# lambdaloop/ucoslam-cv3

Hardware: AMD Instinct MI355X
Metric: tracking frames/sec (ORB extract + match + local BA), 1241x376 mono (higher is better)
Workload: dtype u8 (ORB, Hamming) + f64 (BA); 1 GPU; orb1241x376_2000f_8lv + hamming_knn_2000x10000_nn10 + local_ba_10kf_3000pt; frames_per_keyframe=4

## Files before the change

### ucoslam-cv3_amd/csrc/ba.hip

```cpp
#include <cfloat>
#include <functional>
#include <cstdio>
#include <emmintrin.h>
#include <immintrin.h>
#include <condition_variable>
#include <mutex>
#include <string>
#include <thread>
#include <type_traits>
#include <cmath>
#include <cstdlib>
#include <chrono>
#include <atomic>

#include "common.hpp"
#include "reduce.hpp"

namespace {

constexpr int kMaxFree = 64;
constexpr int kThreads = 256;
constexpr int kSolveThreads = 256;
constexpr int kHbmThreads = 512;
constexpr int kFusedThreads = 512;
// ... 2616 lines not shown
    ResLayout R;
    uh::Layout A;
    R.poses = A.take<float>(16 * (size_t)Kc); R.state = A.take<double>(7 * (size_t)Kc); R.points = A.take<float>(3 * (size_t)Pc);
    R.bad = A.take<unsigned char>(Ec);
    R.bytes_no_chi2 = (A.off + 7) & ~(size_t)7;
    R.chi2 = A.take<double>(Ec);
    R.bytes = (A.off + 7) & ~(size_t)7;
    return R;
}

static int ensure_staging(uh_ba* b, int K, int P, int E) {
    UH_HIP_CHECK(hipSetDevice(b->ctx->device));
    if (b->stage_in_flight) { UH_HIP_CHECK(hipEventSynchronize(b->ev_stage)); b->stage_in_flight = false; }
    if (b->h_stage && K <= b->cap_K && P <= b->cap_P && E <= b->cap_E) return UH_OK;
    const int Kc = K <= b->cap_K ? b->cap_K : K + K / 4 + 4, Pc = P <= b->cap_P ? b->cap_P : P + P / 4 + 64, Ec = E <= b->cap_E ? b->cap_E : E + E / 4 + 1024;
    const StageLayout L = stage_layout(Kc, Pc);
    const ResLayout R = res_layout(Kc, Pc, Ec);
    const size_t bytes = L.obs + (size_t)Ec * sizeof(uh_ba_obs) + 256;
    unsigned char* ns = nullptr; unsigned char* nr = nullptr;
    hipError_t e = hipHostMalloc(reinterpret_cast<void**>(&ns), bytes, hipHostMallocMapped);
    if (e == hipSuccess) e = hipHostMalloc(reinterpret_cast<void**>(&nr), R.bytes + 256, hipHostMallocMapped);
    if (e != hipSuccess) {
        if (ns) (void)hipHostFree(ns);
        uh::set_error("uh_ba: hipHostMalloc of the staging / result blocks (%zu + %zu bytes) failed: %s", bytes, R.bytes, hipGetErrorString(e));
        return UH_ENOMEM;
    }
    if (b->h_stage || b->h_res) UH_HIP_CHECK(hipStreamSynchronize(b->ctx->stream));
    if (b->h_stage) (void)hipHostFree(b->h_stage);
    if (b->h_res) (void)hipHostFree(b->h_res);
    std::memset(nr, 0, R.bytes + 256);
    b->h_stage = ns; b->h_stage_bytes = bytes; b->h_res = nr; b->h_res_bytes = R.bytes + 256;
    b->cap_K = Kc; b->cap_P = Pc; b->cap_E = Ec; b->slay = L; b->rlay = R;
    b->have_problem = false; b->optimized = false;
    if (!b->ev_stage) UH_HIP_CHECK(hipEventCreateWithFlags(&b->ev_stage, hipEventDisableTiming));
    return UH_OK;
}

struct PersistPlan { bool ok; int NF, Lw, G, krows, nelem, SL, max_fix, kfix, lds, nb4, nblk, KS, off_cam; };

template <int NF>
static int persist_lds_bytes(const PersistPlan& pl, int n) { return persist_lds<NF>(pl.krows, n, pl.max_fix, pl.kfix, pl.off_cam, pl.KS, pl.SL).total_bytes; }

static int persist_lanes(int nfree) {
    if (const char* e = getenv("UH_BA_NF")) { const int v = atoi(e); if ((v == 8 || v == 16) && nfree <= v) return v; }
    return nfree <= 8 ? 8 : (nfree <= 16 ? 16 : 0);
}

template <int NF>
static hipError_t persist_grant_lds(int bytes) {
    return hipFuncSetAttribute(reinterpret_cast<const void*>(&ba_persist_kernel<NF>), hipFuncAttributeMaxDynamicSharedMemorySize, bytes);
}

static PersistPlan plan_persistent(uh_ba* b, int K, int P, int E, int nfree) {
    PersistPlan pl{};
    const char* form = getenv("UH_BA_FORM");
    if (form && std::string(form) == "legacy") return pl;
    if (getenv("UH_BA_WIDE") && atoi(getenv("UH_BA_WIDE")) != 0) return pl;
    void* dflag = nullptr;
    if (!b->h_stop || hipHostGetDevicePointer(&dflag, b->h_stop, 0) != hipSuccess) return pl;
    if (nfree < 1 || P < 1 || E >= (1 << 20) - 1) return pl;
    if (b->persist_blocked > 0) { --b->persist_blocked; return pl; }
    const int NF = persist_lanes(nfree);
    if (!NF) return pl;
    const int kLwMax = kPThreads / NF;
    int Lw = std::max(std::min(8, kLwMax), std::min(kLwMax, uh_div_up(P, 64)));
    if (const char* e = getenv("UH_BA_LW")) Lw = std::max(1, std::min(kLwMax, atoi(e)));
    const int G = uh_div_up(P, Lw);
    const int cus = b->ctx->num_cus > 0 ? b->ctx->num_cus : 256;
    if (G > cus) return pl;
    const int kfix = K - nfree;
    if (kfix > 255) return pl;
    pl.NF = NF; pl.Lw = Lw; pl.G = G; pl.kfix = kfix;
    pl.max_fix = Lw * kfix;
    pl.krows = (3 * Lw + 15) & ~15;
    const int n = 6 * nfree;
    pl.nb4 = (n + 3) / 4; pl.nblk = pl.nb4 * (pl.nb4 + 1) / 2;
    pl.off_cam = pl.nblk * 16;
    pl.nelem = pl.off_cam + NF * 27 + 6 * NF + 4;
    pl.SL = (uh_div_up(pl.nelem, G) + 1) & ~1;
    pl.KS = 1;
    {
        int best = 1 << 30;
        for (int ks = 1; ks <= 6; ks++) {
            if (ks > 1 && ks * pl.off_cam > (n + 1) * (n + 1) + 1452) break;
            const int rounds = uh_div_up(pl.nblk * ks, kPThreads), depth = (uh_div_up(pl.krows, ks) + 3) & ~3;
            if (rounds * depth < best) { best = rounds * depth; pl.KS = ks; }
        }
    }
    pl.lds = NF == 8 ? persist_lds_bytes<8>(pl, n) : persist_lds_bytes<16>(pl, n);
    if (b->max_lds <= 0) {
        int v = 0;
        if (hipDeviceGetAttribute(&v, hipDeviceAttributeMaxSharedMemoryPerBlock, b->ctx->device) != hipSuccess || v <= 0) v = 64 * 1024;
        b->max_lds = v;
    }
    if (pl.lds > b->max_lds) return pl;
    const int cls = NF == 8 ? 0 : 1;
    if (pl.lds > b->p_lds_set[cls]) {
        if ((NF == 8 ? persist_grant_lds<8>(pl.lds) : persist_grant_lds<16>(pl.lds)) != hipSuccess) { (void)hipGetLastError(); return pl; }
        b->p_lds_set[cls] = pl.lds;
    }
    pl.ok = true;
    return pl;
}

__attribute__((target("avx512f,avx512vl,avx512dq"))) static int pack_obs16_avx512(const int32_t* pt_, const int32_t* kf_, const float* uv_, const double* w_, int e0, int e1, int P, int K,
                                                                                 unsigned char* ob, bool& exact_out, unsigned& oob) {
    const __m256i pmax = _mm256_set1_epi32(P - 1), kmax = _mm256_set1_epi32(K - 1);
    __m256i bad = _mm256_setzero_si256();
    __mmask8 exact = 0xFF;
    const __m512i idx0 = _mm512_setr_epi32(0, 16, 17, 8, 1, 18, 19, 9, 2, 20, 21, 10, 3, 22, 23, 11);
    const __m512i idx1 = _mm512_setr_epi32(4, 24, 25, 12, 5, 26, 27, 13, 6, 28, 29, 14, 7, 30, 31, 15);
    int i = e0;
    unsigned char* dst = ob + 16 * (size_t)e0;
    for (; i + 8 <= e1; i += 8, dst += 128) {
        const __m256i pt = _mm256_loadu_si256(reinterpret_cast<const __m256i*>(pt_ + i));
        const __m256i kf = _mm256_loadu_si256(reinterpret_cast<const __m256i*>(kf_ + i));
        const __m512 uv = _mm512_loadu_ps(uv_ + 2 * i);
        const __m512d w = _mm512_loadu_pd(w_ + i);
        bad = _mm256_or_si256(bad, _mm256_or_si256(_mm256_or_si256(pt, _mm256_sub_epi32(pmax, pt)), _mm256_or_si256(kf, _mm256_sub_epi32(kmax, kf))));
        const __m256 wf = _mm512_cvtpd_ps(w);
        exact &= _mm512_cmp_pd_mask(_mm512_cvtps_pd(wf), w, _CMP_EQ_OQ);
        const __m256i pk = _mm256_or_si256(pt, _mm256_slli_epi32(kf, 24));
        const __m512 a = _mm512_insertf32x8(_mm512_castps256_ps512(_mm256_castsi256_ps(pk)), wf, 1);
        _mm512_storeu_ps(dst, _mm512_permutex2var_ps(a, idx0, uv));
        _mm512_storeu_ps(dst + 64, _mm512_permutex2var_ps(a, idx1, uv));
    }
    if (exact != 0xFF) exact_out = false;
    oob |= _mm256_movemask_ps(_mm256_castsi256_ps(bad)) ? 1u : 0u;
    return i - e0;
}

using ObsPacker = std::function<void(int, int, bool, bool&, unsigned&)>;
static int set_problem_fast(uh_ba* b, int K, int P, int E, const PersistPlan& pl, bool obs16 = false, const ObsPacker* pack = nullptr, unsigned* oob_out = nullptr) {
    const StageLayout& L = b->slay;
    unsigned char* hs = b->h_stage;
    const float* poses = reinterpret_cast<const float*>(hs + L.poses_in);
    const unsigned char* fixed = hs + L.fixed;
    const float* intr_f = reinterpret_cast<const float*>(hs + L.intr_f);
    double* pose0 = reinterpret_cast<double*>(hs + L.pose0); double* R0 = reinterpret_cast<double*>(hs + L.poseR0);
    double* intr = reinterpret_cast<double*>(hs + L.intr);
    int* slot = reinterpret_cast<int*>(hs + L.slot); int* free_kf = reinterpret_cast<int*>(hs + L.free_kf); int* fix_kf = reinterpret_cast<int*>(hs + L.fix_kf);
    int nfree = 0, nfix = 0;
    for (int k = 0; k < K; k++) {
        if (!fixed[k]) { slot[k] = nfree; free_kf[nfree++] = k; } else { slot[k] = -1; fix_kf[nfix++] = k; }
        const float* M = poses + 16 * k;
        const double R[9] = {M[0], M[1], M[2], M[4], M[5], M[6], M[8], M[9], M[10]};
        double* qq = pose0 + 7 * k;
        quat_from_R_host(R, qq);
        qq[4] = M[3]; qq[5] = M[7]; qq[6] = M[11];
        for (int j = 0; j < 4; j++) intr[4 * k + j] = intr_f[4 * k + j];
        double* Rk = R0 + 12 * k;
        const double tx = 2 * qq[0], ty = 2 * qq[1], tz = 2 * qq[2];
        const double twx = tx * qq[3], twy = ty * qq[3], twz = tz * qq[3];
        const double txx = tx * qq[0], txy = ty * qq[0], txz = tz * qq[0];
        const double tyy = ty * qq[1], tyz = tz * qq[1], tzz = tz * qq[2];
        Rk[0] = 1 - (tyy + tzz); Rk[1] = txy - twz; Rk[2] = txz + twy;
        Rk[3] = txy + twz; Rk[4] = 1 - (txx + tzz); Rk[5] = tyz - twx;
        Rk[6] = txz - twy; Rk[7] = tyz + twx; Rk[8] = 1 - (txx + tyy);
        Rk[9] = qq[4]; Rk[10] = qq[5]; Rk[11] = qq[6];
    }
    UH_HIP_CHECK(hipSetDevice(b->ctx->device));
    hipStream_t st = b->ctx->stream;
    int rc;
    if ((rc = b->dstage.reserve(b->h_stage_bytes))) return rc;
    if ((rc = b->dT.reserve((size_t)P * K * sizeof(unsigned) + 256))) return rc;
    if (b->dT_gen != b->dT.gen || (b->tseq & 0xFFFu) == 0xFFFu) {
        UH_HIP_CHECK(hipMemsetAsync(b->dT.p, 0, b->dT.cap, st));
        b->dT_gen = b->dT.gen; b->tseq = 0;
    }
// ... 568 lines not shown
```

### ucoslam-cv3_amd/csrc/ba_persist.hpp

```cpp
#pragma once

#pragma clang fp contract(fast)

constexpr int kPThreads = 256;
constexpr int kPWaves = kPThreads / 64;
constexpr long long kPTimeoutTicksDefault = 10000000ll;

struct BAPersist {
    int G, Lw, krows, SL, nelem, max_fix, kfix;
    int nb4, nblk, KS;
    int n1, n2, stop_at_begin;
    int speculate;
    unsigned launch_id;
    long long timeout_ticks;
    unsigned tag_base;
    float minChi2;
    const unsigned* T; unsigned tseq;
    const uh_ba_obs* obs;
    int obs16;
    const float* points;
    const float* poses_in;
    const int* fix_kf;
    const double* pose0; const double* poseR0;
    float* r_poses; double* r_state; float* r_points; unsigned char* r_bad; double* r_chi2;
    int want_chi2;
    unsigned long long* r_dev; unsigned long long* r_host; size_t r_words;
    unsigned* done_ctr; unsigned done_base;
    unsigned long long* part;
    unsigned long long* red;
    unsigned long long* partC;
    BAState* host_state;
    unsigned long long* host_done;
    unsigned long long* errw;
};

constexpr int kFxCam = 20;
struct PersistLds {
    int Yt, U, usz, out, wsum, x, bp, bs, bsp, wv, pose, poseR, red, sc, fxchi, fxobs, fxcam, fxact_bytes, fxk_bytes, fxid_bytes, fxptr_bytes, pair_bytes, blk_bytes, flag_bytes, total_bytes;
};
template <int NF>
__host__ __device__ inline PersistLds persist_lds(int krows, int n, int max_fix, int kfix, int off_cam, int KS, int SL) {
    constexpr int NP = 6 * NF, YS = NP + 2;
    PersistLds o;
    int a = 0;
    o.Yt = a; a += krows * YS;
    o.U = a;
    o.usz = (n + 1) * (n + 1) + (n + 1 <= 64 ? 2 * 121 * 6 : 2 * 6 * 128 + 4);
    if (o.usz < KS * off_cam) o.usz = KS * off_cam;
    { const int r = KS * off_cam + (SL > 256 ? SL : 256) + 8; if (o.usz < r) o.usz = r; }
    if (o.usz < kPWaves * NF * 33) o.usz = kPWaves * NF * 33;
    if (o.usz < 2048) o.usz = 2048;
    a += o.usz;
    o.out = a; a += NF * 27 + NP + 4;
    o.wsum = a; a += kPWaves * NF * 33;
    o.x = a; a += NP; o.bp = a; a += NP; o.bs = a; a += NP;
    o.bsp = a; a += kPWaves * NP;
    o.wv = a; a += krows;
    o.pose = a; a += 2 * NF * 7; o.poseR = a; a += 2 * NF * 12;
    o.red = a; a += 16; o.sc = a; a += 8;
    o.fxchi = a; a += max_fix;
    o.fxobs = a; a += 3 * max_fix;
    o.fxcam = a; a += kFxCam * kfix;
    o.fxact_bytes = a * 8;
    int b = o.fxact_bytes + ((max_fix + 15) & ~15);
    o.fxk_bytes = b; b += (max_fix + 15) & ~15;
    o.fxid_bytes = b; b += 4 * ((max_fix + 3) & ~3);
    o.fxptr_bytes = b; b += 4 * (kPThreads / NF + 4);
    o.pair_bytes = b; b += NF * (NF + 1) / 2 * 4;
    b = (b + 15) & ~15;
    o.blk_bytes = b; b += ((NP / 4) * (NP / 4 + 1) / 2 * 2 + 15) & ~15;
    o.flag_bytes = b; b += 16;
    o.total_bytes = b;
    return o;
}

typedef unsigned long long pword;
struct TWord { pword lo, hi; };
__device__ __forceinline__ void tst(pword* base, size_t i, double v, unsigned tag) {
    const pword b = (pword)__double_as_longlong(v);
    typedef unsigned int u32x4 __attribute__((ext_vector_type(4)));
    const u32x4 w = {(unsigned)b, tag, (unsigned)(b >> 32), tag};
    const __amdgpu_buffer_rsrc_t rs = __builtin_amdgcn_make_buffer_rsrc(base, 0, 0x7FFFFFFF, 0x00020000);
    __builtin_amdgcn_raw_buffer_store_b128(w, rs, (int)(i * 16), 0, 16);
}
__device__ __forceinline__ TWord tld_raw(const pword* base, size_t i) {
    TWord w;
    w.lo = __hip_atomic_load(base + 2 * i, __ATOMIC_RELAXED, __HIP_MEMORY_SCOPE_AGENT);
    w.hi = __hip_atomic_load(base + 2 * i + 1, __ATOMIC_RELAXED, __HIP_MEMORY_SCOPE_AGENT);
    return w;
}
__device__ __forceinline__ bool tok(const TWord& w, unsigned tag) { return (unsigned)(w.lo >> 32) == tag && (unsigned)(w.hi >> 32) == tag; }
__device__ __forceinline__ double tval(const TWord& w) { return __longlong_as_double((long long)((w.hi << 32) | (w.lo & 0xffffffffull))); }

__device__ __forceinline__ double rsqrt_nr(double x) {
    double r = __builtin_amdgcn_rsq(x);
    r = r * fma(-0.5 * x, r * r, 1.5);
    r = r * fma(-0.5 * x, r * r, 1.5);
    return r;
}

template <int JAC>
__device__ __forceinline__ void edge_eval_p(double u, double v, double w, double fx, double fy, double cx, double cy, double delta, double dsqr,
                                            const double* Rt, const double* X, bool robust, EdgeLin& o) {
    const double x = Rt[0] * X[0] + Rt[1] * X[1] + Rt[2] * X[2] + Rt[9];
    const double y = Rt[3] * X[0] + Rt[4] * X[1] + Rt[5] * X[2] + Rt[10];
    const double z = Rt[6] * X[0] + Rt[7] * X[1] + Rt[8] * X[2] + Rt[11];
    const double iz = fast_rcp(z);
    const double xz = x * iz, yz = y * iz;
    o.ex = u - (xz * fx + cx);
    o.ey = v - (yz * fy + cy);
    o.chi2 = w * (o.ex * o.ex + o.ey * o.ey);
    o.rho1 = 1.0;
    o.robchi = o.chi2;
    if (robust && o.chi2 > dsqr) {
        const double rs = rsqrt_nr(o.chi2);
        o.rho1 = delta * rs;
        o.robchi = 2 * (o.chi2 * rs) * delta - dsqr;
    }
    if (JAC >= 1) {
        o.ww = o.rho1 * w;
        o.r0 = -w * o.ex * o.rho1;
        o.r1 = -w * o.ey * o.rho1;
        const double fxz = fx * iz, fyz = fy * iz;
#pragma unroll
        for (int c = 0; c < 3; c++) {
            o.A[c] = -fxz * (Rt[c] - xz * Rt[6 + c]);
            o.A[3 + c] = -fyz * (Rt[3 + c] - yz * Rt[6 + c]);
        }
        if (JAC >= 2) {
            o.B[0] = xz * yz * fx; o.B[1] = -(1 + xz * xz) * fx; o.B[2] = yz * fx; o.B[3] = -fxz; o.B[4] = 0; o.B[5] = xz * fxz;
            o.B[6] = (1 + yz * yz) * fy; o.B[7] = -xz * yz * fy; o.B[8] = -xz * fy; o.B[9] = 0; o.B[10] = -fyz; o.B[11] = yz * fyz;
        }
// ... 238 lines not shown
    for (int i = tid; i < kPWaves * NP; i += kPThreads) s_bsp[i] = 0.0;
    for (int i = tid; i < NF * 27 + NP + 4; i += kPThreads) s_out[i] = 0.0;
    for (int i = tid; i < 2 * NF * 7; i += kPThreads) s_pose[i] = 0.0;
    for (int i = tid; i < 2 * NF * 12; i += kPThreads) s_poseR[i] = 0.0;
    if (tid < 8) s_sc[tid] = 0.0;
    __syncthreads();
    if (tid < nl) {
        int c = 0;
        for (int j = 0; j < q.kfix; j++) c += cell(l0 + tid, q.fix_kf[j]) >= 0;
        s_fxptr[tid + 1] = c;
    }
    if (tid == 0) s_fxptr[0] = 0;
    __syncthreads();
    if (tid == 0) for (int i = 0; i < nl; i++) s_fxptr[i + 1] += s_fxptr[i];
    __syncthreads();
    if (tid < nl) {
        int at = s_fxptr[tid];
        for (int j = 0; j < q.kfix; j++) {
            const int e = cell(l0 + tid, q.fix_kf[j]);
            if (e < 0) continue;
            double fu, fv, fw;
            load_obs(e, fu, fv, fw);
            s_fxact[at] = 1; s_fxchi[at] = 0.0; s_fxk[at] = (unsigned char)j; s_fxid[at] = e;
            s_fxobs[3 * at] = fu; s_fxobs[3 * at + 1] = fv; s_fxobs[3 * at + 2] = fw;
            ++at;
        }
    }
    for (int i = tid; i < q.kfix * kFxCam; i += kPThreads) {
        const int f = i / kFxCam, j = i - f * kFxCam, k = q.fix_kf[f];
        s_fxcam[i] = j < 12 ? q.poseR0[12 * k + j] : (j < 16 ? p.intr[4 * k + (j - 12)] : (double)q.poses_in[16 * (size_t)k + 8 + (j - 16)]);
    }
    const int fxb = live ? s_fxptr[ll] : 0, fxe = live ? s_fxptr[ll + 1] : 0;
    if (tid < nfree) {
        const int k = p.free_kf[tid];
        for (int b = 0; b < 2; b++) {
            for (int j = 0; j < 7; j++) s_pose[(b * NF + tid) * 7 + j] = q.pose0[7 * k + j];
            for (int j = 0; j < 12; j++) s_poseR[(b * NF + tid) * 12 + j] = q.poseR0[12 * k + j];
        }
    }
    for (int t = tid; t < npairs; t += kPThreads) {
        int s1 = 0, rem = t;
        while (rem >= nfree - s1) { rem -= nfree - s1; ++s1; }
        s_pair[t][0] = (short)s1; s_pair[t][1] = (short)(s1 + rem);
    }
    for (int t = tid; t < q.nblk; t += kPThreads) {
        int bi = 0, rem = t;
        while (rem >= q.nb4 - bi) { rem -= q.nb4 - bi; ++bi; }
        s_blk[t][0] = (unsigned char)bi; s_blk[t][1] = (unsigned char)(bi + rem);
    }
    if (tid == 0) { s_flag[0] = 1; s_flag[1] = 0; s_flag[2] = 0; }
    __syncthreads();

    unsigned ep = 0, tagA = 0;
    auto next_tag = [&]() -> unsigned { ++ep; return q.tag_base | (ep & 0xFFFu); };
    const pword err_word = ((pword)q.launch_id << 32) | 1ull;
    auto give_up = [&](long long& t0) -> bool {
        if (t0 < 63) { ++t0; return false; }
        if (t0 == 63) t0 = wall_clock64();
        if (__hip_atomic_load(q.errw, __ATOMIC_RELAXED, __HIP_MEMORY_SCOPE_AGENT) == err_word || wall_clock64() - t0 > q.timeout_ticks) {
            s_flag[1] = 1;
            __hip_atomic_store(q.errw, err_word, __ATOMIC_RELAXED, __HIP_MEMORY_SCOPE_AGENT);
            if (q.host_done) __hip_atomic_store(q.host_done, ((unsigned long long)q.launch_id << 32) | 2ull, __ATOMIC_RELEASE, __HIP_MEMORY_SCOPE_SYSTEM);
            return true;
        }
        __builtin_amdgcn_s_sleep(1);
        return false;
    };
    auto tload8 = [&](const pword* base, size_t first, size_t stride, int cnt, unsigned tag, double (&v)[8], unsigned need = 0xFFu) {
        long long t0 = 0;
        for (;;) {
            TWord w[8];
            bool ok = true;
#pragma unroll
            for (int u = 0; u < 8; u++) if (u < cnt && ((need >> u) & 1u)) w[u] = tld_raw(base, first + u * stride);
#pragma unroll
            for (int u = 0; u < 8; u++) { if (u < cnt && ((need >> u) & 1u)) { ok = ok && tok(w[u], tag); v[u] = tval(w[u]); } else v[u] = 0.0; }
            if (ok || give_up(t0)) return;
        }
    };
    const unsigned sl_inv = (unsigned)(0x100000000ull / (unsigned)SL) + 1u;
    auto div_sl = [&](int i) -> int { return (int)__umulhi((unsigned)i, sl_inv); };
    auto part_at = [&](int i) -> size_t { const int sl = div_sl(i); return ((size_t)sl * G + g) * SL + (i - sl * SL); };

    auto prod_index = [&](int row, int col) -> int {
        const int bi = row >> 2, bj = col >> 2;
        return (bi * q.nb4 - bi * (bi - 1) / 2 + (bj - bi)) * 16 + (row & 3) * 4 + (col & 3);
    };
    auto is_diag_elem = [&](int idx) -> bool {
        if (idx >= OFF_CAM) return false;
        int row, col;
        const int bq = idx >> 4;
        row = 4 * s_blk[bq][0] + ((idx >> 2) & 3); col = 4 * s_blk[bq][1] + (idx & 3);
        return row == col && col < n;
    };
    int fold_i[2], fold_s[2];
#pragma unroll
    for (int u = 0; u < 2; u++) {
        const int t = tid + u * kPThreads;
        fold_i[u] = -1; fold_s[u] = 0;
        if (t < nfree * 21) {
            const int sc = t / 21, qq = t - 21 * sc;
            int a = 0, rem = qq;
            while (rem >= 6 - a) { rem -= 6 - a; ++a; }
            fold_i[u] = prod_index(6 * sc + a, 6 * sc + a + rem);
            fold_s[u] = sc * 27 + qq;
        }
    }
    const bool red_diag0 = tid < SL && is_diag_elem(g * SL + tid);
    const int open_beg = div_sl(OFF_CAM) * SL;
    const int red_HG = max(1, min(G, kPThreads / SL));
    const unsigned hg_inv = (unsigned)(0x100000000ull / (unsigned)red_HG) + 1u;
    bool clk_on = false;
    int n_kept = 0, n_dropped = 0;
#define UH_BA_CLKT(i) do { if (clk_on) UH_BA_CLK(i); } while (0)
    BAState st;
    memset(&st, 0, sizeof(st));
    st.phase = 2; st.lambda = -1; st.ni = 2;
    bool robust = true;
    double chi_lin_pass = 0;

    double acc[10];
    double hp[33];
    double H[18];
    bool any = false;
    auto lin_eval = [&](int buf, const double (&Xp)[3], bool first) {
#pragma unroll
        for (int i = 0; i < 10; i++) acc[i] = 0;
#pragma unroll
        for (int i = 0; i < 33; i++) hp[i] = 0;
#pragma unroll
        for (int i = 0; i < 18; i++) H[i] = 0;
        any = false;
        const bool on = has && act;
        if (on) {
            EdgeLin L;
            edge_eval_p<2>(ou, ov, ow, fxk, fyk, cxk, cyk, d.delta, d.dsqr, s_poseR + (buf * NF + s) * 12, Xp, robust, L);
            any = true;
            if (first) chi_e = L.chi2;
            acc[9] = L.robchi;
            acc[0] = L.ww * (L.A[0] * L.A[0] + L.A[3] * L.A[3]); acc[1] = L.ww * (L.A[0] * L.A[1] + L.A[3] * L.A[4]);
            acc[2] = L.ww * (L.A[0] * L.A[2] + L.A[3] * L.A[5]); acc[3] = L.ww * (L.A[1] * L.A[1] + L.A[4] * L.A[4]);
            acc[4] = L.ww * (L.A[1] * L.A[2] + L.A[4] * L.A[5]); acc[5] = L.ww * (L.A[2] * L.A[2] + L.A[5] * L.A[5]);
            acc[6] = L.A[0] * L.r0 + L.A[3] * L.r1; acc[7] = L.A[1] * L.r0 + L.A[4] * L.r1; acc[8] = L.A[2] * L.r0 + L.A[5] * L.r1;
#pragma unroll
            for (int a = 0; a < 6; a++)
#pragma unroll
                for (int c = 0; c < 3; c++) H[a * 3 + c] = L.ww * (L.B[a] * L.A[c] + L.B[6 + a] * L.A[3 + c]);
            int qq = 0;
#pragma unroll
            for (int a = 0; a < 6; a++)
#pragma unroll
                for (int c = a; c < 6; c++) hp[qq++] = L.ww * (L.B[a] * L.B[c] + L.B[6 + a] * L.B[6 + c]);
#pragma unroll
            for (int a = 0; a < 6; a++) hp[21 + a] = L.B[a] * L.r0 + L.B[6 + a] * L.r1;
        }
        {
            for (int i = fxb + s; i < fxe; i += NF) {
                if (!s_fxact[i]) continue;
                any = true;
                const double* C = s_fxcam + kFxCam * s_fxk[i];
                EdgeLin L;
                edge_eval_p<1>(s_fxobs[3 * i], s_fxobs[3 * i + 1], s_fxobs[3 * i + 2], C[12], C[13], C[14], C[15], d.delta, d.dsqr, C, Xp, robust, L);
                if (first) s_fxchi[i] = L.chi2;
                acc[9] += L.robchi;
                acc[0] += L.ww * (L.A[0] * L.A[0] + L.A[3] * L.A[3]); acc[1] += L.ww * (L.A[0] * L.A[1] + L.A[3] * L.A[4]);
                acc[2] += L.ww * (L.A[0] * L.A[2] + L.A[3] * L.A[5]); acc[3] += L.ww * (L.A[1] * L.A[1] + L.A[4] * L.A[4]);
                acc[4] += L.ww * (L.A[1] * L.A[2] + L.A[4] * L.A[5]); acc[5] += L.ww * (L.A[2] * L.A[2] + L.A[5] * L.A[5]);
                acc[6] += L.A[0] * L.r0 + L.A[3] * L.r1; acc[7] += L.A[1] * L.r0 + L.A[4] * L.r1; acc[8] += L.A[2] * L.r0 + L.A[5] * L.r1;
            }
        }
    };
    auto phase1 = [&](double lambda, bool first, double scale_lane, double stop_val) {
        tagA = next_tag();
        if (!first) UH_BA_CLKT(52);
#pragma unroll
        for (int i = 0; i < 10; i++) acc[i] = group_sum<NF>(acc[i]);
        const unsigned long long anym = __ballot(any);
        any_pt = ((anym >> (lane & ~(NF - 1))) & ((1ull << NF) - 1)) != 0;
        bl0 = acc[6]; bl1 = acc[7]; bl2 = acc[8];
        if (first) {
        } else if (any_pt) {
            const double d00 = acc[0] + lambda, d11 = acc[3] + lambda, d22 = acc[5] + lambda;
            ci00 = rsqrt_nr(d00);
            cl10 = acc[1] * ci00; cl20 = acc[2] * ci00;
            ci11 = rsqrt_nr(d11 - cl10 * cl10);
            cl21 = (acc[4] - cl20 * cl10) * ci11;
            ci22 = rsqrt_nr(d22 - cl20 * cl20 - cl21 * cl21);
            wl0 = bl0 * ci00;
            wl1 = (bl1 - cl10 * wl0) * ci11;
            wl2 = (bl2 - cl20 * wl0 - cl21 * wl1) * ci22;
        } else {
            ci00 = ci11 = ci22 = cl10 = cl20 = cl21 = wl0 = wl1 = wl2 = 0;
        }
        if (!first && 3 * ll + 2 < q.krows) {
#pragma unroll
            for (int a = 0; a < 6; a++) {
                const double y0 = H[a * 3] * ci00;
                const double y1 = (H[a * 3 + 1] - cl10 * y0) * ci11;
                const double y2 = (H[a * 3 + 2] - cl20 * y0 - cl21 * y1) * ci22;
                Yt[(3 * ll) * YS + 6 * s + a] = y0; Yt[(3 * ll + 1) * YS + 6 * s + a] = y1; Yt[(3 * ll + 2) * YS + 6 * s + a] = y2;
                hp[27 + a] = y0 * wl0 + y1 * wl1 + y2 * wl2;
            }
        }
        {
            int off = 0, real = 33;
            PartTranspose<33, 32, NF>::run(hp, lane, off, real);
#pragma unroll
            for (int i = 0; i < NHP; i++) if (i < real) s_wsum[(wv * NF + s) * 33 + off + i] = hp[i];
        }
        if (!first) UH_BA_CLKT(53);
        const double chi_part = (live && s == 0) ? acc[9] : 0.0;
        const double maxd = (live && s == 0 && any_pt) ? fmax(fabs(acc[0]), fmax(fabs(acc[3]), fabs(acc[5]))) : 0.0;
        double cs = chi_part, mx = maxd, ss = scale_lane;
        block_reduce3<kPWaves>(cs, mx, ss, s_red);
        for (int t = tid; t < NF * 33; t += kPThreads) {
            double r = s_wsum[t];
#pragma unroll
            for (int w = 1; w < kPWaves; w++) r += s_wsum[w * NF * 33 + t];
            const int sc = t / 33, i = t - 33 * sc;
            s_out[i < 27 ? sc * 27 + i : NF * 27 + 6 * sc + (i - 27)] = r;
        }
        if (tid == 0) { s_out[NF * 27 + NP] = cs; s_out[NF * 27 + NP + 1] = ss; s_out[NF * 27 + NP + 2] = mx; s_out[NF * 27 + NP + 3] = g == 0 ? stop_val : 0.0; }
        if (!first) UH_BA_CLKT(54);
        if (!first) {
            const int nitems = q.nblk * q.KS;
            const int kc = (q.krows + q.KS - 1) / q.KS;
            for (int item = tid; item < nitems; item += kPThreads) {
                const int kt = item / q.nblk, bq = item - kt * q.nblk;
                const int bi = s_blk[bq][0], bj = s_blk[bq][1];
                const int kbeg = kt * kc, kend = min(q.krows, kbeg + kc);
                double acc4[16];
#pragma unroll
                for (int i = 0; i < 16; i++) acc4[i] = 0;
                const double* ra = Yt + 4 * bi, * rb = Yt + 4 * bj;
                for (int k = kbeg; k < kend; k += 4) {
                    double2 a01[4], a23[4], b01[4], b23[4];
#pragma unroll
                    for (int u = 0; u < 4; u++) {
                        const int kk = k + u < kend ? k + u : kbeg;
                        a01[u] = *reinterpret_cast<const double2*>(ra + kk * YS); a23[u] = *reinterpret_cast<const double2*>(ra + kk * YS + 2);
                        b01[u] = *reinterpret_cast<const double2*>(rb + kk * YS); b23[u] = *reinterpret_cast<const double2*>(rb + kk * YS + 2);
                    }
#pragma unroll
                    for (int u = 0; u < 4; u++) {
                        const double z = k + u < kend ? 1.0 : 0.0;
                        const double av[4] = {a01[u].x * z, a01[u].y * z, a23[u].x * z, a23[u].y * z}, bv[4] = {b01[u].x, b01[u].y, b23[u].x, b23[u].y};
#pragma unroll
                        for (int r = 0; r < 4; r++)
#pragma unroll
                            for (int c = 0; c < 4; c++) acc4[r * 4 + c] = fma(av[r], bv[c], acc4[r * 4 + c]);
                    }
                }
#pragma unroll
                for (int i = 0; i < 16; i++) U[kt * OFF_CAM + bq * 16 + i] = acc4[i];
            }
        }
        if (!first) UH_BA_CLKT(55);
        __syncthreads();
        if (!first) UH_BA_CLKT(56);
        if (!first) {
#pragma unroll
            for (int u = 0; u < 2; u++) if (fold_i[u] >= 0) U[fold_i[u]] -= s_out[fold_s[u]];
            for (int j = tid; j < n; j += kPThreads) { const int sc = j / 6; s_out[NF * 27 + j] -= s_out[sc * 27 + 21 + (j - 6 * sc)]; }
        }
        __syncthreads();
        if (!first) UH_BA_CLKT(60);
        for (int i = tid; i < NF * 27 + NP + 4; i += kPThreads) {
            if (!first && i < NF * 27 && i - 27 * (i / 27) < 21) continue;
            tst(q.part, part_at(OFF_CAM + i), s_out[i], tagA);
        }
        if (!first) UH_BA_CLKT(61);
        const int KSs = q.KS;
        for (int i = (first ? open_beg : 0) + tid; i < OFF_CAM; i += kPThreads) {
            double r = 0.0;
            if (!first) { r = U[i]; for (int kt = 1; kt < KSs; kt++) r += U[kt * OFF_CAM + i]; }
            tst(q.part, part_at(i), r, tagA);
        }
    };

    unsigned tagB = 0;
    auto reduce_slices = [&](double lam, bool first) -> bool {
        tagB = next_tag();
        const int HG = red_HG;
        double* const R = U + q.KS * OFF_CAM;
        const size_t src = (size_t)g * G * SL;
        for (int idx = tid; idx < SL * HG; idx += kPThreads) {
            const int hg = div_sl(idx), e = idx - hg * SL;
            const bool is_max = g * SL + e == OFF_SC + 2;
            const int ge = g * SL + e;
            const bool hpp = ge >= OFF_CAM && ge < OFF_BS && (ge - OFF_CAM) - 27 * ((ge - OFF_CAM) / 27) < 21;
            const bool used = ge < q.nelem && !(first && (g + 1) * SL <= OFF_CAM) && !(hpp && !first);
            double r = 0.0;
            bool have = false;
            for (int h = hg; used && h < G; h += 8 * HG) {
                double v[8];
                const int cnt = min(8, HG == 1 ? G - h : (int)__umulhi((unsigned)(G - h + HG - 1), hg_inv));
                tload8(q.part, src + (size_t)h * SL + e, (size_t)HG * SL, cnt, tagA, v);
#pragma unroll
                for (int u = 0; u < 8; u++) {
                    if (u >= cnt) continue;
                    r = !have ? v[u] : (is_max ? fmax(r, v[u]) : r + v[u]);
                    have = true;
                }
            }
            R[idx] = r;
        }
        UH_BA_CLKT(50);
        __syncthreads();
        if (s_flag[1]) return false;
        for (int e = tid; e < SL; e += kPThreads) {
            const bool is_max = g * SL + e == OFF_SC + 2;
            double r = R[e];
            for (int hg = 1; hg < HG; hg++) { const double v = R[hg * SL + e]; r = is_max ? fmax(r, v) : r + v; }
            if (e == tid ? red_diag0 : is_diag_elem(g * SL + e)) r -= lam;
            {
                const int ge = g * SL + e;
                if (!first && ge >= OFF_CAM && ge < OFF_BS && (ge - OFF_CAM) - 27 * ((ge - OFF_CAM) / 27) < 21) continue;
            }
            tst(q.red, (size_t)g * SL + e, r, tagB);
        }
        UH_BA_CLKT(51);
        __syncthreads();
        return true;
    };

    auto dst_of = [&](int idx) -> int {
        int t = -1;
        if (idx < q.nelem) {
            if (idx < OFF_CAM) {
                int row, col;
                const int bq = idx >> 4, rr = (idx >> 2) & 3, cq = idx & 3;
                row = 4 * s_blk[bq][0] + rr; col = 4 * s_blk[bq][1] + cq;
                if (row <= col && col < n) t = o.U + col * ld + row;
            } else if (idx < OFF_BS) {
                const int i = idx - OFF_CAM, sc = i / 27, k = i - 27 * sc;
                if (k >= 21) t = (o.bp + 6 * sc + (k - 21)) | (1 << 24);
            } else if (idx < OFF_SC) t = o.U + n * ld + (idx - OFF_BS);
            else t = (o.sc + 4 + (idx - OFF_SC)) | (1 << 24);
        }
        return t;
    };
    int asm_dst[8];
#pragma unroll
    for (int u = 0; u < 8; u++) asm_dst[u] = dst_of(tid + u * kPThreads);
    UH_BA_CLK(1);
    for (int pass = 0; pass < 2; pass++) {
        UH_BA_CLK(2 + 3 * pass);
        if (pass == 1) {
            if (st.stopped) break;
            st.gate = 1;
            st.iters_pass1 = st.iters_done;
            if (has) {
                const double* Rt = s_poseR + (st.cur * NF + s) * 12;
                const double z = Rt[6] * X[0] + Rt[7] * X[1] + Rt[8] * X[2] + Rt[11];
                if (chi_e > d.chi2_th || !(z > 0.0)) act = false;
            }
            for (int i = fxb + s; i < fxe; i += NF) {
                const double* Rt = s_fxcam + kFxCam * s_fxk[i];
                const double z = Rt[6] * X[0] + Rt[7] * X[1] + Rt[8] * X[2] + Rt[11];
                if (s_fxchi[i] > d.chi2_th || !(z > 0.0)) s_fxact[i] = 0;
            }
            robust = false;
            __syncthreads();
        }
        const int max_iters = pass == 0 ? q.n1 : q.n2;
        st.pending = 0; st.stop_seen = 0;
        st.phase = max_iters > 0 ? 0 : 2;
// ... 302 lines not shown
```

Baseline: 9187 frames/s.

## Restructure persistent BA Schur block products into per-wave K-split with shuffle reduction

Replaces the flat item loop that wrote each K-slice of every 4x4 block product into LDS and then summed slices after a block barrier. Each wave now owns a group of blocks, with lanes split across K slices. Partial sums are combined by wavefront shuffles, staged in a small per-wave LDS buffer, and streamed straight to the global partial buffer. The camera-diagonal fold is precomputed into a compact Hb buffer during the wsum reduction, and the KS selection cost model is changed to match. The aim is to cut LDS footprint and block-wide syncs and to overlap global stores with compute; the price is more complex indexing and wave-level fences, which carry correctness risk.

```diff
diff --git a/ucoslam-cv3_amd/csrc/ba.hip b/ucoslam-cv3_amd/csrc/ba.hip
--- a/ucoslam-cv3_amd/csrc/ba.hip
+++ b/ucoslam-cv3_amd/csrc/ba.hip
@@ -2722,9 +2722,10 @@
     {
         int best = 1 << 30;
         for (int ks = 1; ks <= 6; ks++) {
-            if (ks > 1 && ks * pl.off_cam > (n + 1) * (n + 1) + 1452) break;
-            const int rounds = uh_div_up(pl.nblk * ks, kPThreads), depth = (uh_div_up(pl.krows, ks) + 3) & ~3;
-            if (rounds * depth < best) { best = rounds * depth; pl.KS = ks; }
+            const int bpw = std::min(64 / ks, uh_div_up(pl.nblk, kPWaves));
+            const int rounds = uh_div_up(pl.nblk, kPWaves * bpw), depth = (uh_div_up(pl.krows, ks) + 3) & ~3;
+            const int cost = rounds * (depth + (ks - 1) + 4);
+            if (cost < best) { best = cost; pl.KS = ks; }
         }
     }
     pl.lds = NF == 8 ? persist_lds_bytes<8>(pl, n) : persist_lds_bytes<16>(pl, n);
diff --git a/ucoslam-cv3_amd/csrc/ba_persist.hpp b/ucoslam-cv3_amd/csrc/ba_persist.hpp
--- a/ucoslam-cv3_amd/csrc/ba_persist.hpp
+++ b/ucoslam-cv3_amd/csrc/ba_persist.hpp
@@ -4,6 +4,7 @@
 
 constexpr int kPThreads = 256;
 constexpr int kPWaves = kPThreads / 64;
+constexpr bool kCameraSideFirst = false;
 constexpr long long kPTimeoutTicksDefault = 10000000ll;
 
 struct BAPersist {
@@ -36,7 +37,7 @@
 
 constexpr int kFxCam = 20;
 struct PersistLds {
-    int Yt, U, usz, out, wsum, x, bp, bs, bsp, wv, pose, poseR, red, sc, fxchi, fxobs, fxcam, fxact_bytes, fxk_bytes, fxid_bytes, fxptr_bytes, pair_bytes, blk_bytes, flag_bytes, total_bytes;
+    int Yt, U, usz, bpw, hb, rscr, out, wsum, x, bp, bs, bsp, wv, pose, poseR, red, sc, fxchi, fxobs, fxcam, fxact_bytes, fxk_bytes, fxid_bytes, fxptr_bytes, pair_bytes, blk_bytes, flag_bytes, total_bytes;
 };
 template <int NF>
 __host__ __device__ inline PersistLds persist_lds(int krows, int n, int max_fix, int kfix, int off_cam, int KS, int SL) {
@@ -46,8 +47,16 @@
     o.Yt = a; a += krows * YS;
     o.U = a;
     o.usz = (n + 1) * (n + 1) + (n + 1 <= 64 ? 2 * 121 * 6 : 2 * 6 * 128 + 4);
-    if (o.usz < KS * off_cam) o.usz = KS * off_cam;
-    { const int r = KS * off_cam + (SL > 256 ? SL : 256) + 8; if (o.usz < r) o.usz = r; }
+    {
+        const int nblk = off_cam / 16, nb4 = (n + 3) / 4, per = (nblk + kPWaves - 1) / kPWaves;
+        o.bpw = 64 / KS < per ? 64 / KS : per;
+        const int scr = (SL > 256 ? SL : 256) + 8, hbsz = 2 * nb4 * 16;
+        const int cap = o.usz > KS * off_cam + scr ? o.usz : KS * off_cam + scr;
+        while (o.bpw > 1 && kPWaves * o.bpw * 16 + hbsz + scr > cap) --o.bpw;
+        o.hb = kPWaves * o.bpw * 16;
+        o.rscr = o.hb + hbsz;
+        if (o.usz < o.rscr + scr) o.usz = o.rscr + scr;
+    }
     if (o.usz < kPWaves * NF * 33) o.usz = kPWaves * NF * 33;
     if (o.usz < 2048) o.usz = 2048;
     a += o.usz;
@@ -452,10 +461,6 @@
     auto div_sl = [&](int i) -> int { return (int)__umulhi((unsigned)i, sl_inv); };
     auto part_at = [&](int i) -> size_t { const int sl = div_sl(i); return ((size_t)sl * G + g) * SL + (i - sl * SL); };
 
-    auto prod_index = [&](int row, int col) -> int {
-        const int bi = row >> 2, bj = col >> 2;
-        return (bi * q.nb4 - bi * (bi - 1) / 2 + (bj - bi)) * 16 + (row & 3) * 4 + (col & 3);
-    };
     auto is_diag_elem = [&](int idx) -> bool {
         if (idx >= OFF_CAM) return false;
         int row, col;
@@ -463,19 +468,33 @@
         row = 4 * s_blk[bq][0] + ((idx >> 2) & 3); col = 4 * s_blk[bq][1] + (idx & 3);
         return row == col && col < n;
     };
-    int fold_i[2], fold_s[2];
-#pragma unroll
-    for (int u = 0; u < 2; u++) {
-        const int t = tid + u * kPThreads;
-        fold_i[u] = -1; fold_s[u] = 0;
-        if (t < nfree * 21) {
-            const int sc = t / 21, qq = t - 21 * sc;
+    double* const Hb = U + o.hb;
+    constexpr int NSUM = (NF * 33 + kPThreads - 1) / kPThreads, NHZ = (2 * (NP / 4) * 16 + kPThreads - 1) / kPThreads;
+    int hb_i[NSUM];
+    unsigned hb_zero = 0;
+#pragma unroll
+    for (int u = 0; u < NSUM; u++) {
+        const int t = tid + u * kPThreads, sc = t / 33, qq = t - 33 * sc;
+        hb_i[u] = -1;
+        if (sc < nfree && qq < 21) {
             int a = 0, rem = qq;
             while (rem >= 6 - a) { rem -= 6 - a; ++a; }
-            fold_i[u] = prod_index(6 * sc + a, 6 * sc + a + rem);
-            fold_s[u] = sc * 27 + qq;
-        }
-    }
+            const int row = 6 * sc + a, col = row + rem, bi = row >> 2, bj = col >> 2;
+            hb_i[u] = ((bj - bi) * q.nb4 + bi) * 16 + (row & 3) * 4 + (col & 3);
+        }
+    }
+#pragma unroll
+    for (int u = 0; u < NHZ; u++) {
+        const int t = tid + u * kPThreads;
+        if (t < 2 * q.nb4 * 16) {
+            const int dd = t >= q.nb4 * 16 ? 1 : 0, bi = (t >> 4) - dd * q.nb4;
+            const int row = 4 * bi + ((t >> 2) & 3), col = 4 * (bi + dd) + (t & 3);
+            if (!(row <= col && col < n && row / 6 == col / 6)) hb_zero |= 1u << u;
+        }
+    }
+    const int p_kt = lane / o.bpw, p_bl = lane - p_kt * o.bpw;
+    const int p_kc = ((q.krows + q.KS - 1) / q.KS + 3) & ~3;
+    const int p_kbeg = min(q.krows, p_kt * p_kc), p_kend = p_kt < q.KS ? min(q.krows, p_kbeg + p_kc) : p_kbeg;
     const bool red_diag0 = tid < SL && is_diag_elem(g * SL + tid);
     const int open_beg = div_sl(OFF_CAM) * SL;
     const int red_HG = max(1, min(G, kPThreads / SL));
@@ -583,76 +602,127 @@
         const double maxd = (live && s == 0 && any_pt) ? fmax(fabs(acc[0]), fmax(fabs(acc[3]), fabs(acc[5]))) : 0.0;
         double cs = chi_part, mx = maxd, ss = scale_lane;
         block_reduce3<kPWaves>(cs, mx, ss, s_red);
-        for (int t = tid; t < NF * 33; t += kPThreads) {
+#pragma unroll
+        for (int u = 0; u < NSUM; u++) {
+            const int t = tid + u * kPThreads;
+            if (t >= NF * 33) break;
             double r = s_wsum[t];
 #pragma unroll
             for (int w = 1; w < kPWaves; w++) r += s_wsum[w * NF * 33 + t];
             const int sc = t / 33, i = t - 33 * sc;
-            s_out[i < 27 ? sc * 27 + i : NF * 27 + 6 * sc + (i - 27)] = r;
+            if (i < 27) {
+                s_out[sc * 27 + i] = r;
+                if (!first && hb_i[u] >= 0) Hb[hb_i[u]] = r;
+            } else {
+                if (!first && sc < nfree) {
+                    double rp = s_wsum[t - 6];
+#pragma unroll
+                    for (int w = 1; w < kPWaves; w++) rp += s_wsum[w * NF * 33 + t - 6];
+                    r -= rp;
+                }
+                s_out[NF * 27 + 6 * sc + (i - 27)] = r;
+            }
+        }
+        if (!first) {
+#pragma unroll
+            for (int u = 0; u < NHZ; u++) if ((hb_zero >> u) & 1u) Hb[tid + u * kPThreads] = 0.0;
         }
         if (tid == 0) { s_out[NF * 27 + NP] = cs; s_out[NF * 27 + NP + 1] = ss; s_out[NF * 27 + NP + 2] = mx; s_out[NF * 27 + NP + 3] = g == 0 ? stop_val : 0.0; }
+        __syncthreads();
         if (!first) UH_BA_CLKT(54);
-        if (!first) {
-            const int nitems = q.nblk * q.KS;
-            const int kc = (q.krows + q.KS - 1) / q.KS;
-            for (int item = tid; item < nitems; item += kPThreads) {
-                const int kt = item / q.nblk, bq = item - kt * q.nblk;
-                const int bi = s_blk[bq][0], bj = s_blk[bq][1];
-                const int kbeg = kt * kc, kend = min(q.krows, kbeg + kc);
-                double acc4[16];
-#pragma unroll
-                for (int i = 0; i < 16; i++) acc4[i] = 0;
-                const double* ra = Yt + 4 * bi, * rb = Yt + 4 * bj;
-                for (int k = kbeg; k < kend; k += 4) {
-                    double2 a01[4], a23[4], b01[4], b23[4];
-#pragma unroll
-                    for (int u = 0; u < 4; u++) {
-                        const int kk = k + u < kend ? k + u : kbeg;
-                        a01[u] = *reinterpret_cast<const double2*>(ra + kk * YS); a23[u] = *reinterpret_cast<const double2*>(ra + kk * YS + 2);
-                        b01[u] = *reinterpret_cast<const double2*>(rb + kk * YS); b23[u] = *reinterpret_cast<const double2*>(rb + kk * YS + 2);
-                    }
-#pragma unroll
-                    for (int u = 0; u < 4; u++) {
-                        const double z = k + u < kend ? 1.0 : 0.0;
-                        const double av[4] = {a01[u].x * z, a01[u].y * z, a23[u].x * z, a23[u].y * z}, bv[4] = {b01[u].x, b01[u].y, b23[u].x, b23[u].y};
-#pragma unroll
-                        for (int r = 0; r < 4; r++)
-#pragma unroll
-                            for (int c = 0; c < 4; c++) acc4[r * 4 + c] = fma(av[r], bv[c], acc4[r * 4 + c]);
-                    }
+        auto send_camera_side = [&]() {
+            for (int i = tid; i < NF * 27 + NP + 4; i += kPThreads) {
+                if (!first && i < NF * 27 && i - 27 * (i / 27) < 21) continue;
+                tst(q.part, part_at(OFF_CAM + i), s_out[i], tagA);
+            }
+        };
+        if (first || kCameraSideFirst) send_camera_side();
+        if (!first) UH_BA_CLKT(60);
+        if (first) {
+            for (int i = open_beg + tid; i < OFF_CAM; i += kPThreads) tst(q.part, part_at(i), 0.0, tagA);
+            return;
+        }
+        double* const stg = U + wvu * (o.bpw * 16);
+        for (int b0 = wvu * o.bpw; b0 < q.nblk; b0 += kPWaves * o.bpw) {
+            const bool on = p_kt < q.KS && b0 + p_bl < q.nblk;
+            const int bq = on ? b0 + p_bl : 0;
+            const int bi = s_blk[bq][0], bj = s_blk[bq][1];
+            const int kend = on ? p_kend : p_kbeg;
+            double acc4[16];
+#pragma unroll
+            for (int i = 0; i < 16; i++) acc4[i] = 0;
+            const double* ra = Yt + 4 * bi, * rb = Yt + 4 * bj;
+            double2 s0[8], s1[8];
+            auto load2 = [&](double2 (&st2)[8], int k) {
+#pragma unroll
+                for (int u = 0; u < 2; u++) {
+                    st2[4 * u] = *reinterpret_cast<const double2*>(ra + (k + u) * YS); st2[4 * u + 1] = *reinterpret_cast<const double2*>(ra + (k + u) * YS + 2);
+                    st2[4 * u + 2] = *reinterpret_cast<const double2*>(rb + (k + u) * YS); st2[4 * u + 3] = *reinterpret_cast<const double2*>(rb + (k + u) * YS + 2);
                 }
-#pragma unroll
-                for (int i = 0; i < 16; i++) U[kt * OFF_CAM + bq * 16 + i] = acc4[i];
-            }
-        }
-        if (!first) UH_BA_CLKT(55);
-        __syncthreads();
-        if (!first) UH_BA_CLKT(56);
-        if (!first) {
-#pragma unroll
-            for (int u = 0; u < 2; u++) if (fold_i[u] >= 0) U[fold_i[u]] -= s_out[fold_s[u]];
-            for (int j = tid; j < n; j += kPThreads) { const int sc = j / 6; s_out[NF * 27 + j] -= s_out[sc * 27 + 21 + (j - 6 * sc)]; }
-        }
-        __syncthreads();
-        if (!first) UH_BA_CLKT(60);
-        for (int i = tid; i < NF * 27 + NP + 4; i += kPThreads) {
-            if (!first && i < NF * 27 && i - 27 * (i / 27) < 21) continue;
-            tst(q.part, part_at(OFF_CAM + i), s_out[i], tagA);
+            };
+            auto fma2 = [&](const double2 (&st2)[8]) {
+#pragma unroll
+                for (int u = 0; u < 2; u++) {
+                    const double av[4] = {st2[4 * u].x, st2[4 * u].y, st2[4 * u + 1].x, st2[4 * u + 1].y}, bv[4] = {st2[4 * u + 2].x, st2[4 * u + 2].y, st2[4 * u + 3].x, st2[4 * u + 3].y};
+#pragma unroll
+                    for (int r = 0; r < 4; r++)
+#pragma unroll
+                        for (int c = 0; c < 4; c++) acc4[r * 4 + c] = fma(av[r], bv[c], acc4[r * 4 + c]);
+                }
+            };
+            if (p_kbeg < kend) load2(s0, p_kbeg);
+            for (int k = p_kbeg; k < kend; k += 4) {
+                load2(s1, k + 2);
+                __builtin_amdgcn_sched_barrier(0);
+                fma2(s0);
+                __builtin_amdgcn_sched_barrier(0);
+                load2(s0, k + 4 < kend ? k + 4 : k);
+                __builtin_amdgcn_sched_barrier(0);
+                fma2(s1);
+                __builtin_amdgcn_sched_barrier(0);
+            }
+            if (!first) UH_BA_CLKT(55);
+            double sum4[16];
+#pragma unroll
+            for (int i = 0; i < 16; i++) sum4[i] = acc4[i];
+            if (on && p_kt == 0 && bj - bi <= 1) {
+                const double2* hb = reinterpret_cast<const double2*>(Hb + ((bj - bi) * q.nb4 + bi) * 16);
+#pragma unroll
+                for (int i = 0; i < 8; i++) { const double2 h = hb[i]; sum4[2 * i] -= h.x; sum4[2 * i + 1] -= h.y; }
+            }
+            for (int kt = 1; kt < q.KS; kt++) {
+                const int src = (lane + kt * o.bpw) & 63;
+                double sh[16];
+#pragma unroll
+                for (int i = 0; i < 16; i++) sh[i] = __shfl(acc4[i], src);
+                __builtin_amdgcn_sched_barrier(0);
+#pragma unroll
+                for (int i = 0; i < 16; i++) sum4[i] += sh[i];
+                __builtin_amdgcn_sched_barrier(0);
+            }
+            __builtin_amdgcn_fence(__ATOMIC_RELEASE, "wavefront");
+            __builtin_amdgcn_wave_barrier();
+            if (on && p_kt == 0) {
+                double2* sd = reinterpret_cast<double2*>(stg + p_bl * 16);
+#pragma unroll
+                for (int i = 0; i < 8; i++) sd[i] = make_double2(sum4[2 * i], sum4[2 * i + 1]);
+            }
+            __builtin_amdgcn_fence(__ATOMIC_RELEASE, "wavefront");
+            __builtin_amdgcn_wave_barrier();
+            __builtin_amdgcn_fence(__ATOMIC_ACQUIRE, "wavefront");
+            if (!first) UH_BA_CLKT(56);
+            const int cnt = min(o.bpw, q.nblk - b0) * 16;
+            for (int e = lane; e < cnt; e += 64) tst(q.part, part_at(b0 * 16 + e), stg[e], tagA);
         }
         if (!first) UH_BA_CLKT(61);
-        const int KSs = q.KS;
-        for (int i = (first ? open_beg : 0) + tid; i < OFF_CAM; i += kPThreads) {
-            double r = 0.0;
-            if (!first) { r = U[i]; for (int kt = 1; kt < KSs; kt++) r += U[kt * OFF_CAM + i]; }
-            tst(q.part, part_at(i), r, tagA);
-        }
+        if (!kCameraSideFirst) send_camera_side();
     };
 
     unsigned tagB = 0;
     auto reduce_slices = [&](double lam, bool first) -> bool {
         tagB = next_tag();
         const int HG = red_HG;
-        double* const R = U + q.KS * OFF_CAM;
+        double* const R = U + o.rscr;
         const size_t src = (size_t)g * G * SL;
         for (int idx = tid; idx < SL * HG; idx += kPThreads) {
             const int hg = div_sl(idx), e = idx - hg * SL;
```

Measured after the change: 9079 frames/s. 1.2% lower.
